# tl32rodan/DCVC

Hardware: AMD Instinct MI355X
Metric: encode+decode fps @1920x1080 per GPU; bpp bit-exact + PSNR Δ<1e-4 dB vs ref (higher is better)
Workload: dtype f32 (convs on split-fp16 f16x3 MFMA, fp32 accumulation); 1 GPU; C3 DCVC-DC RGB 1920x1080 (pad 1920x1088) IP=32 write mode; gop=32, precision=split, q_index=0, stream_part=8, parallelism=sequence-sharded x1, 3 GOP lane(s) per GPU, lanes=3, step=one frame on each of 3 lane(s)

## Files before the change

### dcvc_amd/csrc/hip/sdc.hip

```cpp
#include "common.h"
#include "launch.h"
#include "split.h"

namespace {

constexpr int kNW = 8, kNT = kNW * 64;
constexpr int TH = 8, TW = 16;
constexpr int HW_ = TW + 2, NPH = (TH + 2) * HW_;
constexpr int HR = 192;

struct DP {
  const float *x;
  int H, W, xcs, xco;
  float *y;
  int ycs, yco;
  const uint16_t *w;
  int wbytes;
  const float *b1, *wdw, *bdw, *b2, *ba;
  float slope;
  int tiles_x, ntiles;
  int *ovf;
};

template <int CIN, int COUT, bool ADAPT>
struct DG {
  static constexpr int KCI = (CIN + 31) / 32;
  static constexpr int NTI = (CIN + 15) / 16, NTO = (COUT + 15) / 16;
  static constexpr int CI16 = NTI * 16, CO16 = NTO * 16;
  static constexpr int W1 = KCI * CI16 * 32, W2 = KCI * CO16 * 32, WA = ADAPT ? KCI * CO16 * 32 : 0;
  static constexpr int NWH = 2 * (W1 + W2 + WA);
  static constexpr int XI = KCI * HR * 32;
  static constexpr int DI = KCI * TH * TW * 32;
  static constexpr size_t OX = 0, OD = OX + (size_t)2 * XI * 2, OW = OD + (size_t)2 * DI * 2;
  static constexpr size_t OC = OW + (size_t)NWH * 2;
  static constexpr int NC = CIN * 11 + 2 * COUT;
  static constexpr size_t LDS = OC + (size_t)NC * 4;
  static constexpr int QP = CIN / 8;
  static constexpr int PP = (NPH * QP + kNT - 1) / kNT;
};

__device__ __forceinline__ float lrelu(float v, float s) { return fmaxf(v, v * s); }

template <int CIN, int COUT, bool ADAPT>
__global__ void __launch_bounds__(kNT) sdc_kernel(DP p) {
  SplitRange rg(p.ovf);
  typedef DG<CIN, COUT, ADAPT> G_;
  constexpr int KCI = G_::KCI, NTI = G_::NTI, NTO = G_::NTO, CO16 = G_::CO16, CI16 = G_::CI16;
  constexpr int XI = G_::XI, DI = G_::DI, QP = G_::QP, PP = G_::PP;
  extern __shared__ __align__(16) unsigned char smem[];
  uint16_t *Xh = reinterpret_cast<uint16_t *>(smem + G_::OX), *Xl = Xh + XI;
  uint16_t *Dh = reinterpret_cast<uint16_t *>(smem + G_::OD), *Dl = Dh + DI;
  uint16_t *W1h = reinterpret_cast<uint16_t *>(smem + G_::OW), *W1l = W1h + G_::W1;
  uint16_t *W2h = W1l + G_::W1, *W2l = W2h + G_::W2;
  uint16_t *WAh = W2l + G_::W2, *WAl = WAh + G_::WA;
  float *Lb1 = reinterpret_cast<float *>(smem + G_::OC), *Lbdw = Lb1 + CIN, *Lwdw = Lbdw + CIN;
  float *Lb2 = Lwdw + 9 * CIN, *Lba = Lb2 + COUT;
  auto t1p = [&](int r, int c) -> float * {
    return reinterpret_cast<float *>((c & 16) ? Xl : Xh) + (((c >> 5) * HR + r) * 16 + (c & 15));
  };

  const int tid = threadIdx.x;
  const int wave = tid >> 6, lane = tid & 63;
  const int col = lane & 15, hi = lane >> 4;
  const int G = gridDim.x;
  int g = blockIdx.x;
  if ((G & 7) == 0) g = (g & 7) * (G >> 3) + (g >> 3);
  if (g >= p.ntiles) return;

  {
    const __amdgpu_buffer_rsrc_t wr =
        __builtin_amdgcn_make_buffer_rsrc(const_cast<uint16_t *>(p.w), (short)0, p.wbytes, 0x00020000);
    constexpr int ND = G_::NWH * 2 / 1024;
    for (int i = wave; i < ND; i += kNW)
      __builtin_amdgcn_raw_ptr_buffer_load_lds(wr, (__attribute__((address_space(3))) void *)(W1h + i * 512), 16,
                                               i * 1024 + lane * 16, 0, 0, 0);
    for (int i = tid; i < G_::NC; i += kNT) {
      float v;
      if (i < CIN) v = p.b1[i];
      else if (i < 2 * CIN) v = p.bdw[i - CIN];
      else if (i < 11 * CIN) v = p.wdw[i - 2 * CIN];
      else if (i < 11 * CIN + COUT) v = p.b2[i - 11 * CIN];
      else v = ADAPT ? p.ba[i - 11 * CIN - COUT] : 0.f;
      Lb1[i] = v;
    }
  }

  const __amdgpu_buffer_rsrc_t xr = __builtin_amdgcn_make_buffer_rsrc(
      const_cast<float *>(p.x), (short)0,
      (int)((int64_t)p.H * p.W * p.xcs * 4 < 0x7fff0000 ? (int64_t)p.H * p.W * p.xcs * 4 : 0x7fff0000), 0x00020000);
  int pyx[PP], prel[PP], pofs[PP];
#pragma unroll
  for (int u = 0; u < PP; ++u) {
    const int it = tid + u * kNT;
    pyx[u] = -1;
    prel[u] = 0;
    pofs[u] = 0;
    if (it < NPH * QP) {
      const int pix = it / QP, q = it - pix * QP;
      const int hy = pix / HW_, hx = pix - hy * HW_;
      pyx[u] = (hy << 8) | hx;
      prel[u] = ((hy - 1) * p.W + (hx - 1)) * p.xcs + p.xco + q * 8;
      pofs[u] = swz((q >> 2) * HR + pix, q & 3);
    }
  }
  float pf[PP][8];
  auto prefetch = [&](int t) {
    const int oy0 = (t / p.tiles_x) * TH, ox0 = (t % p.tiles_x) * TW;
    const int base = oy0 * p.W + ox0;
#pragma unroll
    for (int u = 0; u < PP; ++u) {
      const int gy = oy0 - 1 + (pyx[u] >> 8), gx = ox0 - 1 + (pyx[u] & 255);
      const bool in = pyx[u] >= 0 && (unsigned)gy < (unsigned)p.H && (unsigned)gx < (unsigned)p.W;
      const int o = in ? (base * p.xcs + prel[u]) * 4 : 0x7fffffe0;
      const f32x4 a = __builtin_bit_cast(f32x4, __builtin_amdgcn_raw_buffer_load_b128(xr, o, 0, 0));
      const f32x4 b = __builtin_bit_cast(f32x4, __builtin_amdgcn_raw_buffer_load_b128(xr, o + 16, 0, 0));
#pragma unroll
      for (int j = 0; j < 4; ++j) {
        pf[u][j] = a[j];
        pf[u][4 + j] = b[j];
      }
    }
  };
  prefetch(g);

  auto zero_pad = [&]() {
    if constexpr (CIN % 32 != 0) {
      constexpr int PADQ = KCI * 4 - QP;
      for (int it = tid; it < HR * PADQ; it += kNT) {
        const int row = it / PADQ, q = QP + it % PADQ;
        const int o = swz((q >> 2) * HR + row, q & 3);
        *reinterpret_cast<u32x4_t *>(Xh + o) = u32x4_t{0u, 0u, 0u, 0u};
        *reinterpret_cast<u32x4_t *>(Xl + o) = u32x4_t{0u, 0u, 0u, 0u};
      }
    }
  };

  wait_vm_lgkm();
  for (int t = g; t < p.ntiles; t += G) {
    const int oy0 = (t / p.tiles_x) * TH, ox0 = (t % p.tiles_x) * TW;
    raw_barrier();
#pragma unroll
    for (int u = 0; u < PP; ++u) {
      u32x4_t h, l;
      rg.add8(pf[u]);
      split8(pf[u], h, l);
      if (pyx[u] >= 0) {
        *reinterpret_cast<u32x4_t *>(Xh + pofs[u]) = h;
        *reinterpret_cast<u32x4_t *>(Xl + pofs[u]) = l;
      }
    }
    zero_pad();
    wait_lgkm();
    raw_barrier();
    if (t + G < p.ntiles) prefetch(t + G);

    f32x4 idn[NTO];
    if constexpr (ADAPT) {
      f32x4 am[NTO], ac[NTO];
#pragma unroll
      for (int j = 0; j < NTO; ++j) {
        am[j] = f32x4{0.f, 0.f, 0.f, 0.f};
        ac[j] = f32x4{0.f, 0.f, 0.f, 0.f};
      }
      const int hr = (wave + 1) * HW_ + 1 + col;
#pragma unroll
      for (int kc = 0; kc < KCI; ++kc) {
        const int ob = swz(kc * HR + hr, hi);
        const f16x8 bh = *reinterpret_cast<const f16x8 *>(Xh + ob), bl = *reinterpret_cast<const f16x8 *>(Xl + ob);
#pragma unroll
        for (int j = 0; j < NTO; ++j) {
          const int oa = swz(kc * CO16 + j * 16 + col, hi);
          const f16x8 ah = *reinterpret_cast<const f16x8 *>(WAh + oa), al = *reinterpret_cast<const f16x8 *>(WAl + oa);
          am[j] = __builtin_amdgcn_mfma_f32_16x16x32_f16(ah, bh, am[j], 0, 0, 0);
          ac[j] = __builtin_amdgcn_mfma_f32_16x16x32_f16(ah, bl, ac[j], 0, 0, 0);
          ac[j] = __builtin_amdgcn_mfma_f32_16x16x32_f16(al, bh, ac[j], 0, 0, 0);
        }
      }
#pragma unroll
      for (int j = 0; j < NTO; ++j) {
        const int n = j * 16 + hi * 4;
#pragma unroll
        for (int e = 0; e < 4; ++e) idn[j][e] = (am[j][e] + ac[j][e] * kLoInv) + Lba[n + e < COUT ? n + e : 0];
      }
      wait_lgkm();
      raw_barrier();
    }

    for (int ht = wave; ht < HR / 16; ht += kNW) {
      f32x4 tm[NTI], tc[NTI];
#pragma unroll
      for (int j = 0; j < NTI; ++j) {
        tm[j] = f32x4{0.f, 0.f, 0.f, 0.f};
        tc[j] = f32x4{0.f, 0.f, 0.f, 0.f};
      }
      const int r = ht * 16 + col;
#pragma unroll
      for (int kc = 0; kc < KCI; ++kc) {
        const int ob = swz(kc * HR + r, hi);
        const f16x8 bh = *reinterpret_cast<const f16x8 *>(Xh + ob), bl = *reinterpret_cast<const f16x8 *>(Xl + ob);
#pragma unroll
        for (int j = 0; j < NTI; ++j) {
          const int oa = swz(kc * CI16 + j * 16 + col, hi);
          const f16x8 ah = *reinterpret_cast<const f16x8 *>(W1h + oa), al = *reinterpret_cast<const f16x8 *>(W1l + oa);
          tm[j] = __builtin_amdgcn_mfma_f32_16x16x32_f16(ah, bh, tm[j], 0, 0, 0);
          tc[j] = __builtin_amdgcn_mfma_f32_16x16x32_f16(ah, bl, tc[j], 0, 0, 0);
          tc[j] = __builtin_amdgcn_mfma_f32_16x16x32_f16(al, bh, tc[j], 0, 0, 0);
        }
      }
      const int hy = r / HW_, hx = r - hy * HW_;
      const int gy = oy0 - 1 + hy, gx = ox0 - 1 + hx;
      const bool inside = r < NPH && (unsigned)gy < (unsigned)p.H && (unsigned)gx < (unsigned)p.W;
      wave_lds_sync();
#pragma unroll
      for (int j = 0; j < NTI; ++j) {
        const int n = j * 16 + hi * 4;
        if (n >= CIN) continue;
        f32x4 v;
#pragma unroll
        for (int e = 0; e < 4; ++e) v[e] = inside ? lrelu((tm[j][e] + tc[j][e] * kLoInv) + Lb1[n + e], p.slope) : 0.f;
        *reinterpret_cast<f32x4 *>(t1p(r, n)) = v;
      }
    }
    wait_lgkm();
    raw_barrier();

    {
      constexpr int CG = CIN / 4;
      constexpr int R = kNT / (CG * TW) >= 4 ? 4 : kNT / (CG * TW) >= 2 ? 2 : 1;
      constexpr int RR = TH / R;
      static_assert(CG * TW * R <= kNT && TH % R == 0, "P2 tasks");
      if (tid < CG * TW * R) {
        const int cg = tid % CG, rest = tid / CG;
        const int ix = rest % TW, y0 = (rest / TW) * RR;
        const int c = cg * 4;
        f32x4 wv[9];
#pragma unroll
        for (int k = 0; k < 9; ++k) wv[k] = *reinterpret_cast<const f32x4 *>(Lwdw + k * CIN + c);
        const float4 bd = *reinterpret_cast<const float4 *>(Lbdw + c);
        f32x4 win[3][3];
#pragma unroll
        for (int r = 0; r < 2; ++r)
#pragma unroll
          for (int dx = 0; dx < 3; ++dx)
            win[r][dx] = *reinterpret_cast<const f32x4 *>(t1p((y0 + r) * HW_ + ix + dx, c));
#pragma unroll
        for (int i = 0; i < RR; ++i) {
#pragma unroll
          for (int dx = 0; dx < 3; ++dx)
            win[(i + 2) % 3][dx] = *reinterpret_cast<const f32x4 *>(t1p((y0 + i + 2) * HW_ + ix + dx, c));
          f32x4 a = f32x4{0.f, 0.f, 0.f, 0.f};
#pragma unroll
          for (int dy = 0; dy < 3; ++dy)
#pragma unroll
            for (int dx = 0; dx < 3; ++dx)
#pragma unroll
              for (int e = 0; e < 4; ++e) a[e] = __builtin_fmaf(wv[dy * 3 + dx][e], win[(i + dy) % 3][dx][e], a[e]);
          float v[4];
          v[0] = a[0] + bd.x;
          v[1] = a[1] + bd.y;
          v[2] = a[2] + bd.z;
          v[3] = a[3] + bd.w;
          rg.add4(v);
          const auto h01 = __builtin_amdgcn_cvt_pkrtz(v[0], v[1]);
          const auto h23 = __builtin_amdgcn_cvt_pkrtz(v[2], v[3]);
          const uint32_t l01 = pk(split_lo(v[0], (float)h01[0]), split_lo(v[1], (float)h01[1]));
          const uint32_t l23 = pk(split_lo(v[2], (float)h23[0]), split_lo(v[3], (float)h23[1]));
          const int px = (y0 + i) * TW + ix;
          const int o = swz((c >> 5) * (TH * TW) + px, (c & 31) >> 3) + (c & 7);
          typedef unsigned int u32x2_t __attribute__((ext_vector_type(2)));
          *reinterpret_cast<u32x2_t *>(Dh + o) = u32x2_t{__builtin_bit_cast(uint32_t, h01), __builtin_bit_cast(uint32_t, h23)};
          *reinterpret_cast<u32x2_t *>(Dl + o) = u32x2_t{l01, l23};
        }
      }
      if constexpr (CIN % 32 != 0) {
        constexpr int PADQ = KCI * 4 - CIN / 8;
        for (int it = tid; it < TH * TW * PADQ; it += kNT) {
          const int px = it / PADQ, q = CIN / 8 + it % PADQ;
          const int o = swz((q >> 2) * (TH * TW) + px, q & 3);
          *reinterpret_cast<u32x4_t *>(Dh + o) = u32x4_t{0u, 0u, 0u, 0u};
          *reinterpret_cast<u32x4_t *>(Dl + o) = u32x4_t{0u, 0u, 0u, 0u};
        }
      }
    }
    wait_lgkm();
    raw_barrier();

    {
      f32x4 cm[NTO], cc[NTO];
#pragma unroll
      for (int j = 0; j < NTO; ++j) {
        cm[j] = f32x4{0.f, 0.f, 0.f, 0.f};
        cc[j] = f32x4{0.f, 0.f, 0.f, 0.f};
      }
#pragma unroll
      for (int kc = 0; kc < KCI; ++kc) {
        const int ob = swz(kc * (TH * TW) + wave * TW + col, hi);
        const f16x8 bh = *reinterpret_cast<const f16x8 *>(Dh + ob), bl = *reinterpret_cast<const f16x8 *>(Dl + ob);
#pragma unroll
        for (int j = 0; j < NTO; ++j) {
          const int oa = swz(kc * CO16 + j * 16 + col, hi);
          const f16x8 ah = *reinterpret_cast<const f16x8 *>(W2h + oa), al = *reinterpret_cast<const f16x8 *>(W2l + oa);
          cm[j] = __builtin_amdgcn_mfma_f32_16x16x32_f16(ah, bh, cm[j], 0, 0, 0);
          cc[j] = __builtin_amdgcn_mfma_f32_16x16x32_f16(ah, bl, cc[j], 0, 0, 0);
          cc[j] = __builtin_amdgcn_mfma_f32_16x16x32_f16(al, bh, cc[j], 0, 0, 0);
        }
      }
      const int gy = oy0 + wave, gx = ox0 + col;
      if (gy < p.H && gx < p.W) {
        const int64_t pix = (int64_t)gy * p.W + gx;
#pragma unroll
        for (int j = 0; j < NTO; ++j) {
          const int n = j * 16 + hi * 4;
          if (n >= COUT) continue;
          f32x4 id;
          if constexpr (ADAPT) id = idn[j];
          else id = *reinterpret_cast<const f32x4 *>(p.x + pix * p.xcs + p.xco + n);
          f32x4 v;
#pragma unroll
          for (int e = 0; e < 4; ++e) v[e] = ((cm[j][e] + cc[j][e] * kLoInv) + Lb2[n + e]) + id[e];
          *reinterpret_cast<f32x4 *>(p.y + pix * p.ycs + p.yco + n) = v;
        }
      }
    }
  }
  wait_vm_lgkm();
}

template <int CIN, int COUT, bool ADAPT>
int run(DP p, hipStream_t st) {
  typedef DG<CIN, COUT, ADAPT> G_;
  static_assert(G_::LDS <= 160 * 1024, "LDS");
  static_assert(G_::NWH * 2 % 1024 == 0, "weight images in whole 1-KiB pieces");
  p.tiles_x = (p.W + TW - 1) / TW;
  const int64_t nt = (int64_t)p.tiles_x * ((p.H + TH - 1) / TH);
  if (nt <= 0) return DCVC_HIP_OK;
  p.ntiles = (int)nt;
  const int cus = dcvc_cu_count();
  if (cus <= 0) return DCVC_HIP_ELAUNCH;
  int G = cus;
  if (G > p.ntiles) G = p.ntiles;
  auto kern = sdc_kernel<CIN, COUT, ADAPT>;
  dcvc_note_kernel("sdc_kernel<%d, %d, %s>@%lld", CIN, COUT, bname(ADAPT), (long long)G * kNT);
  dcvc_ensure_lds(reinterpret_cast<const void *>(kern), (int)G_::LDS);
  hipLaunchKernelGGL(kern, dim3((unsigned)G), dim3(kNT), G_::LDS, st, p);
  DCVC_LAUNCH_CHECK();
  return DCVC_HIP_OK;
}

bool supported(int cin, int cout, bool adapt) {
  return (cin == 64 && cout == 48 && adapt) || (cin == 48 && cout == 32 && adapt) ||
         (cin == 64 && cout == 64 && !adapt) || (cin == 32 && cout == 64 && adapt) ||
         (cin == 48 && cout == 48 && !adapt) || (cin == 32 && cout == 32 && !adapt);
}

}

extern "C" int64_t dcvc_dc_pack_weights(const float *w1, const float *w2, const float *wa, int cin, int cout,
                                        void *out) {
  if (!w1 || !w2 || cin <= 0 || cout <= 0) return DCVC_HIP_EINVAL;
  if (out && (!host_split_range_ok(w1, (int64_t)cin * cin) || !host_split_range_ok(w2, (int64_t)cout * cin) ||
              (wa && !host_split_range_ok(wa, (int64_t)cout * cin))))
    return DCVC_HIP_EINVAL;
  const int kci = (cin + 31) / 32, ci16 = (cin + 15) / 16 * 16, co16 = (cout + 15) / 16 * 16;
  const int64_t n1 = (int64_t)kci * ci16 * 32, n2 = (int64_t)kci * co16 * 32, na = wa ? n2 : 0;
  const int64_t total = 2 * (n1 + n2 + na);
  if (!out) return total;
  uint16_t *o = reinterpret_cast<uint16_t *>(out);
  auto at = [](int row, int k) {
    const int x = (0x1320 >> (((row >> 2) & 3) << 2)) & 3;
    return (int64_t)row * 32 + ((((k >> 3) ^ x) & 3) << 3) + (k & 7);
  };
  auto put = [&](uint16_t *img, int64_t n, const float *w, int rows, int rows16) {
    for (int kc = 0; kc < kci; ++kc)
      for (int r = 0; r < rows16; ++r)
        for (int k = 0; k < 32; ++k) {
          const int ch = kc * 32 + k;
          const float v = (r < rows && ch < cin) ? w[(int64_t)r * cin + ch] : 0.f;
          const int64_t q = at(kc * rows16 + r, k);
          host_split(v, img[q], img[n + q]);
        }
  };
  put(o, n1, w1, cin, ci16);
  put(o + 2 * n1, n2, w2, cout, co16);
  if (wa) put(o + 2 * n1 + 2 * n2, na, wa, cout, co16);
  return total;
}

extern "C" int dcvc_depth_conv_split(const dcvc_dc_args *a, void *stream) {
  if (!a || !a->x.ptr || !a->y.ptr || !a->w || !a->b1 || !a->wdw || !a->bdw || !a->b2) return DCVC_HIP_EINVAL;
  if (a->x.dtype != DCVC_F32 || a->y.dtype != DCVC_F32 || a->x.C != a->cin || a->y.C != a->cout ||
      a->x.H != a->y.H || a->x.W != a->y.W)
    return DCVC_HIP_EINVAL;
  const bool adapt = a->adaptor != 0;
  if (!supported(a->cin, a->cout, adapt) || (adapt && !a->ba)) return DCVC_HIP_EUNSUPPORTED;
  if (!(a->slope >= 0.f && a->slope <= 1.f)) return DCVC_HIP_EUNSUPPORTED;
  if (a->x.cstride % 4 || a->x.coff % 4 || a->y.cstride % 4 || a->y.coff % 4 || ((uintptr_t)a->x.ptr & 15) ||
      ((uintptr_t)a->y.ptr & 15))
    return DCVC_HIP_EUNSUPPORTED;
  if ((int64_t)a->x.H * a->x.W * a->x.cstride * 4 >= 0x7fff0000) return DCVC_HIP_EUNSUPPORTED;
  DP p{};
  p.ovf = dcvc_internal_split_flag();
  p.x = reinterpret_cast<const float *>(a->x.ptr);
  p.H = a->x.H;
  p.W = a->x.W;
  p.xcs = a->x.cstride;
  p.xco = a->x.coff;
  p.y = reinterpret_cast<float *>(a->y.ptr);
  p.ycs = a->y.cstride;
  p.yco = a->y.coff;
  p.w = reinterpret_cast<const uint16_t *>(a->w);
  p.wbytes = (int)(dcvc_dc_pack_weights(reinterpret_cast<const float *>(1), reinterpret_cast<const float *>(1),
                                        adapt ? reinterpret_cast<const float *>(1) : nullptr, a->cin, a->cout,
                                        nullptr) * 2);
  p.b1 = a->b1;
  p.wdw = a->wdw;
  p.bdw = a->bdw;
  p.b2 = a->b2;
  p.ba = a->ba;
  p.slope = a->slope;
  hipStream_t st = reinterpret_cast<hipStream_t>(stream);
  if (a->cin == 64 && a->cout == 48) return run<64, 48, true>(p, st);
  if (a->cin == 48 && a->cout == 32) return run<48, 32, true>(p, st);
  if (a->cin == 32 && a->cout == 64) return run<32, 64, true>(p, st);
  if (a->cin == 64 && a->cout == 64) return run<64, 64, false>(p, st);
  if (a->cin == 48 && a->cout == 48) return run<48, 48, false>(p, st);
  return run<32, 32, false>(p, st);
}
```

Before: 30.60 frames/s.

## Add software-pipelined depth-conv kernel overlapping conv1, depthwise and conv2 across channel groups

```diff
diff --git a/dcvc_amd/csrc/hip/sdc.h b/dcvc_amd/csrc/hip/sdc.h
--- /dev/null
+++ b/dcvc_amd/csrc/hip/sdc.h
@@ -0,0 +1,19 @@
+#pragma once
+#include <hip/hip_runtime.h>
+#include <stdint.h>
+
+struct SdcP {
+  const float *x;
+  int H, W, xcs, xco;
+  float *y;
+  int ycs, yco;
+  const uint16_t *w;
+  int wbytes;
+  const float *b1, *wdw, *bdw, *b2, *ba;
+  float slope;
+  int tiles_x, ntiles;
+  int *ovf;
+  int dbg;
+};
+
+int dcvc_internal_sdc_pipe(int cin, int cout, bool adapt, SdcP p, hipStream_t st);
diff --git a/dcvc_amd/csrc/hip/sdc.hip b/dcvc_amd/csrc/hip/sdc.hip
--- a/dcvc_amd/csrc/hip/sdc.hip
+++ b/dcvc_amd/csrc/hip/sdc.hip
@@ -1,5 +1,7 @@
 #include "common.h"
 #include "launch.h"
+#include "options.h"
+#include "sdc.h"
 #include "split.h"
 
 namespace {
@@ -9,18 +11,7 @@
 constexpr int HW_ = TW + 2, NPH = (TH + 2) * HW_;
 constexpr int HR = 192;
 
-struct DP {
-  const float *x;
-  int H, W, xcs, xco;
-  float *y;
-  int ycs, yco;
-  const uint16_t *w;
-  int wbytes;
-  const float *b1, *wdw, *bdw, *b2, *ba;
-  float slope;
-  int tiles_x, ntiles;
-  int *ovf;
-};
+typedef SdcP DP;
 
 template <int CIN, int COUT, bool ADAPT>
 struct DG {
@@ -44,6 +35,14 @@
 template <int CIN, int COUT, bool ADAPT>
 __global__ void __launch_bounds__(kNT) sdc_kernel(DP p) {
   SplitRange rg(p.ovf);
+#ifdef SDC_DBG
+  const int XD = p.dbg;
+#else
+  constexpr int XD = 0;
+#endif
+  auto barrier = [&]() __attribute__((always_inline)) {
+    if (!(XD & 128)) raw_barrier();
+  };
   typedef DG<CIN, COUT, ADAPT> G_;
   constexpr int KCI = G_::KCI, NTI = G_::NTI, NTO = G_::NTO, CO16 = G_::CO16, CI16 = G_::CI16;
   constexpr int XI = G_::XI, DI = G_::DI, QP = G_::QP, PP = G_::PP;
@@ -138,25 +137,26 @@
   wait_vm_lgkm();
   for (int t = g; t < p.ntiles; t += G) {
     const int oy0 = (t / p.tiles_x) * TH, ox0 = (t % p.tiles_x) * TW;
-    raw_barrier();
+    barrier();
 #pragma unroll
     for (int u = 0; u < PP; ++u) {
       u32x4_t h, l;
       rg.add8(pf[u]);
       split8(pf[u], h, l);
-      if (pyx[u] >= 0) {
+      if (pyx[u] >= 0 && !(XD & 1)) {
         *reinterpret_cast<u32x4_t *>(Xh + pofs[u]) = h;
         *reinterpret_cast<u32x4_t *>(Xl + pofs[u]) = l;
       }
     }
     zero_pad();
     wait_lgkm();
-    raw_barrier();
+    barrier();
     if (t + G < p.ntiles) prefetch(t + G);
 
     f32x4 idn[NTO];
     if constexpr (ADAPT) {
       f32x4 am[NTO], ac[NTO];
+      const int KA = (XD & 2) ? 0 : KCI;
 #pragma unroll
       for (int j = 0; j < NTO; ++j) {
         am[j] = f32x4{0.f, 0.f, 0.f, 0.f};
@@ -164,7 +164,7 @@
       }
       const int hr = (wave + 1) * HW_ + 1 + col;
 #pragma unroll
-      for (int kc = 0; kc < KCI; ++kc) {
+      for (int kc = 0; kc < KA; ++kc) {
         const int ob = swz(kc * HR + hr, hi);
         const f16x8 bh = *reinterpret_cast<const f16x8 *>(Xh + ob), bl = *reinterpret_cast<const f16x8 *>(Xl + ob);
 #pragma unroll
@@ -183,7 +183,7 @@
         for (int e = 0; e < 4; ++e) idn[j][e] = (am[j][e] + ac[j][e] * kLoInv) + Lba[n + e < COUT ? n + e : 0];
       }
       wait_lgkm();
-      raw_barrier();
+      barrier();
     }
 
     for (int ht = wave; ht < HR / 16; ht += kNW) {
@@ -194,8 +194,9 @@
         tc[j] = f32x4{0.f, 0.f, 0.f, 0.f};
       }
       const int r = ht * 16 + col;
-#pragma unroll
-      for (int kc = 0; kc < KCI; ++kc) {
+      const int K1 = (XD & 4) ? 0 : KCI;
+#pragma unroll
+      for (int kc = 0; kc < K1; ++kc) {
         const int ob = swz(kc * HR + r, hi);
         const f16x8 bh = *reinterpret_cast<const f16x8 *>(Xh + ob), bl = *reinterpret_cast<const f16x8 *>(Xl + ob);
 #pragma unroll
@@ -214,7 +215,7 @@
 #pragma unroll
       for (int j = 0; j < NTI; ++j) {
         const int n = j * 16 + hi * 4;
-        if (n >= CIN) continue;
+        if (n >= CIN || (XD & 8)) continue;
         f32x4 v;
 #pragma unroll
         for (int e = 0; e < 4; ++e) v[e] = inside ? lrelu((tm[j][e] + tc[j][e] * kLoInv) + Lb1[n + e], p.slope) : 0.f;
@@ -222,14 +223,14 @@
       }
     }
     wait_lgkm();
-    raw_barrier();
+    barrier();
 
     {
       constexpr int CG = CIN / 4;
       constexpr int R = kNT / (CG * TW) >= 4 ? 4 : kNT / (CG * TW) >= 2 ? 2 : 1;
       constexpr int RR = TH / R;
       static_assert(CG * TW * R <= kNT && TH % R == 0, "P2 tasks");
-      if (tid < CG * TW * R) {
+      if (tid < CG * TW * R && !(XD & 16)) {
         const int cg = tid % CG, rest = tid / CG;
         const int ix = rest % TW, y0 = (rest / TW) * RR;
         const int c = cg * 4;
@@ -283,7 +284,7 @@
       }
     }
     wait_lgkm();
-    raw_barrier();
+    barrier();
 
     {
       f32x4 cm[NTO], cc[NTO];
@@ -292,8 +293,9 @@
         cm[j] = f32x4{0.f, 0.f, 0.f, 0.f};
         cc[j] = f32x4{0.f, 0.f, 0.f, 0.f};
       }
-#pragma unroll
-      for (int kc = 0; kc < KCI; ++kc) {
+      const int K3 = (XD & 32) ? 0 : KCI;
+#pragma unroll
+      for (int kc = 0; kc < K3; ++kc) {
         const int ob = swz(kc * (TH * TW) + wave * TW + col, hi);
         const f16x8 bh = *reinterpret_cast<const f16x8 *>(Dh + ob), bl = *reinterpret_cast<const f16x8 *>(Dl + ob);
 #pragma unroll
@@ -306,7 +308,7 @@
         }
       }
       const int gy = oy0 + wave, gx = ox0 + col;
-      if (gy < p.H && gx < p.W) {
+      if (gy < p.H && gx < p.W && !(XD & 64)) {
         const int64_t pix = (int64_t)gy * p.W + gx;
 #pragma unroll
         for (int j = 0; j < NTO; ++j) {
@@ -346,6 +348,10 @@
   DCVC_LAUNCH_CHECK();
   return DCVC_HIP_OK;
 }
+
+#ifdef SDC_DBG
+DCVC_OPTION("sdc_dbg", g_dbg, 0);
+#endif
 
 bool supported(int cin, int cout, bool adapt) {
   return (cin == 64 && cout == 48 && adapt) || (cin == 48 && cout == 32 && adapt) ||
@@ -419,6 +425,12 @@
   p.ba = a->ba;
   p.slope = a->slope;
   hipStream_t st = reinterpret_cast<hipStream_t>(stream);
+#ifdef SDC_DBG
+  p.dbg = g_dbg;
+#else
+  const int rp = dcvc_internal_sdc_pipe(a->cin, a->cout, adapt, p, st);
+  if (rp != DCVC_HIP_EUNSUPPORTED) return rp;
+#endif
   if (a->cin == 64 && a->cout == 48) return run<64, 48, true>(p, st);
   if (a->cin == 48 && a->cout == 32) return run<48, 32, true>(p, st);
   if (a->cin == 32 && a->cout == 64) return run<32, 64, true>(p, st);
diff --git a/dcvc_amd/csrc/hip/sdcp.hip b/dcvc_amd/csrc/hip/sdcp.hip
--- /dev/null
+++ b/dcvc_amd/csrc/hip/sdcp.hip
@@ -0,0 +1,388 @@
+#include "common.h"
+#include "launch.h"
+#include "options.h"
+#include "sdc.h"
+#include "split.h"
+
+namespace {
+
+constexpr int kNW = 8, kNT = kNW * 64;
+constexpr int TH = 8, TW = 16;
+constexpr int HW_ = TW + 2, NPH = (TH + 2) * HW_;
+constexpr int HR = 192;
+constexpr int TP = TH * TW;
+constexpr int kOob = 0x7fffffe0;
+
+typedef uint32_t u32x2_t __attribute__((ext_vector_type(2)));
+
+template <int CIN, int COUT, bool ADAPT>
+struct PG {
+  static constexpr int KCI = (CIN + 31) / 32;
+  static constexpr int NTI = (CIN + 15) / 16, NTO = (COUT + 15) / 16;
+  static constexpr int CI16 = NTI * 16, CO16 = NTO * 16;
+  static constexpr int W1 = KCI * CI16 * 32, W2 = KCI * CO16 * 32, WA = ADAPT ? KCI * CO16 * 32 : 0;
+  static constexpr int XI = KCI * HR * 32;
+  static constexpr int DI = KCI * TP * 32;
+  static constexpr int TPI = 36;
+  static constexpr int TS = NPH * TPI;
+  static constexpr size_t OX = 0, OD = OX + (size_t)2 * XI * 2, OT = OD + (size_t)2 * DI * 2;
+  static constexpr size_t OW = OT + (size_t)2 * TS * 4;
+  static constexpr size_t OC = OW + (size_t)2 * W1 * 2;
+  static constexpr int NC = CIN * 11 + 2 * COUT;
+  static constexpr size_t LDS = OC + (size_t)NC * 4;
+  static constexpr int QP = CIN / 8;
+  static constexpr int PP = (NPH * QP + kNT - 1) / kNT;
+  static constexpr int NRB = NTO <= 2 ? 2 : 4;
+  static constexpr int NPB = TH / (kNW / NRB);
+  static_assert(COUT % 16 == 0 && CIN % 16 == 0 && NTO <= NRB, "whole channel tiles");
+  static_assert(LDS <= 160 * 1024, "LDS of a CU");
+  static_assert((2 * W1 * 2) % 1024 == 0, "conv1's images in whole 1-KiB pieces");
+};
+
+__device__ __forceinline__ float lrelu(float v, float s) { return fmaxf(v, v * s); }
+
+template <int CIN, int COUT, bool ADAPT>
+__global__ void __launch_bounds__(kNT) sdc_kernel_pipe(SdcP p) {
+  SplitRange rg(p.ovf);
+  typedef PG<CIN, COUT, ADAPT> G_;
+  constexpr int KCI = G_::KCI, NTI = G_::NTI, NTO = G_::NTO, CO16 = G_::CO16, CI16 = G_::CI16;
+  constexpr int XI = G_::XI, DI = G_::DI, QP = G_::QP, PP = G_::PP, NRB = G_::NRB, NPB = G_::NPB;
+  extern __shared__ __align__(16) unsigned char smem[];
+  uint16_t *Xh = reinterpret_cast<uint16_t *>(smem + G_::OX), *Xl = Xh + XI;
+  uint16_t *Dh = reinterpret_cast<uint16_t *>(smem + G_::OD), *Dl = Dh + DI;
+  float *Ts = reinterpret_cast<float *>(smem + G_::OT);
+  uint16_t *W1h = reinterpret_cast<uint16_t *>(smem + G_::OW), *W1l = W1h + G_::W1;
+  float *Lb1 = reinterpret_cast<float *>(smem + G_::OC), *Lbdw = Lb1 + CIN, *Lwdw = Lbdw + CIN;
+  float *Lb2 = Lwdw + 9 * CIN, *Lba = Lb2 + COUT;
+
+  const int tid = threadIdx.x, lane = tid & 63;
+  const int wave = __builtin_amdgcn_readfirstlane(tid >> 6);
+  const int col = lane & 15, hi = lane >> 4;
+  const int rb = wave % NRB, pb0 = (wave / NRB) * NPB;
+  const bool mm = rb < NTO;
+  const int n = rb * 16 + hi * 4;
+  const int G = gridDim.x;
+  int g = blockIdx.x;
+  if ((G & 7) == 0) g = (g & 7) * (G >> 3) + (g >> 3);
+  if (g >= p.ntiles) return;
+
+  const __amdgpu_buffer_rsrc_t wr =
+      __builtin_amdgcn_make_buffer_rsrc(const_cast<uint16_t *>(p.w), (short)0, p.wbytes, 0x00020000);
+  {
+    constexpr int ND = 2 * G_::W1 * 2 / 1024;
+    for (int i = wave; i < ND; i += kNW)
+      __builtin_amdgcn_raw_ptr_buffer_load_lds(wr, (__attribute__((address_space(3))) void *)(W1h + i * 512), 16,
+                                               i * 1024 + lane * 16, 0, 0, 0);
+    for (int i = tid; i < G_::NC; i += kNT) {
+      float v;
+      if (i < CIN) v = p.b1[i];
+      else if (i < 2 * CIN) v = p.bdw[i - CIN];
+      else if (i < 11 * CIN) v = p.wdw[i - 2 * CIN];
+      else if (i < 11 * CIN + COUT) v = p.b2[i - 11 * CIN];
+      else v = ADAPT ? p.ba[i - 11 * CIN - COUT] : 0.f;
+      Lb1[i] = v;
+    }
+    for (int i = tid; i < (2 * XI + 2 * DI) / 8; i += kNT)
+      reinterpret_cast<u32x4_t *>(Xh)[i] = u32x4_t{0u, 0u, 0u, 0u};
+  }
+  f16x8 w2h[KCI], w2l[KCI], wah[KCI], wal[KCI];
+#pragma unroll
+  for (int kc = 0; kc < KCI; ++kc) {
+    const int o = mm ? swz(kc * CO16 + rb * 16 + col, hi) * 2 : kOob;
+    const int o2 = mm ? o + 2 * G_::W1 * 2 : kOob;
+    w2h[kc] = __builtin_bit_cast(f16x8, __builtin_amdgcn_raw_buffer_load_b128(wr, o2, 0, 0));
+    w2l[kc] = __builtin_bit_cast(f16x8, __builtin_amdgcn_raw_buffer_load_b128(wr, mm ? o2 + G_::W2 * 2 : kOob, 0, 0));
+    if constexpr (ADAPT) {
+      const int oa = mm ? o + (2 * G_::W1 + 2 * G_::W2) * 2 : kOob;
+      wah[kc] = __builtin_bit_cast(f16x8, __builtin_amdgcn_raw_buffer_load_b128(wr, oa, 0, 0));
+      wal[kc] = __builtin_bit_cast(f16x8, __builtin_amdgcn_raw_buffer_load_b128(wr, mm ? oa + G_::WA * 2 : kOob, 0, 0));
+    } else {
+      wah[kc] = w2h[kc];
+      wal[kc] = w2l[kc];
+    }
+  }
+
+  const __amdgpu_buffer_rsrc_t xr = __builtin_amdgcn_make_buffer_rsrc(
+      const_cast<float *>(p.x), (short)0,
+      (int)((int64_t)p.H * p.W * p.xcs * 4 < 0x7fff0000 ? (int64_t)p.H * p.W * p.xcs * 4 : 0x7fff0000), 0x00020000);
+  int pyx[PP], prel[PP], pofs[PP];
+#pragma unroll
+  for (int u = 0; u < PP; ++u) {
+    const int it = tid + u * kNT;
+    pyx[u] = -1;
+    prel[u] = 0;
+    pofs[u] = 0;
+    if (it < NPH * QP) {
+      const int pix = it / QP, q = it - pix * QP;
+      const int hy = pix / HW_, hx = pix - hy * HW_;
+      pyx[u] = (hy << 8) | hx;
+      prel[u] = ((hy - 1) * p.W + (hx - 1)) * p.xcs + p.xco + q * 8;
+      pofs[u] = swz((q >> 2) * HR + pix, q & 3);
+    }
+  }
+  float pf[PP][8];
+  auto prefetch = [&](int t) __attribute__((always_inline)) {
+    const int oy0 = (t / p.tiles_x) * TH, ox0 = (t % p.tiles_x) * TW;
+    const int base = oy0 * p.W + ox0;
+#pragma unroll
+    for (int u = 0; u < PP; ++u) {
+      const int gy = oy0 - 1 + (pyx[u] >> 8), gx = ox0 - 1 + (pyx[u] & 255);
+      const bool in = pyx[u] >= 0 && (unsigned)gy < (unsigned)p.H && (unsigned)gx < (unsigned)p.W;
+      const int o = in ? (base * p.xcs + prel[u]) * 4 : kOob;
+      const f32x4 a = __builtin_bit_cast(f32x4, __builtin_amdgcn_raw_buffer_load_b128(xr, o, 0, 0));
+      const f32x4 b = __builtin_bit_cast(f32x4, __builtin_amdgcn_raw_buffer_load_b128(xr, o + 16, 0, 0));
+#pragma unroll
+      for (int j = 0; j < 4; ++j) {
+        pf[u][j] = a[j];
+        pf[u][4 + j] = b[j];
+      }
+    }
+  };
+  auto publish = [&]() __attribute__((always_inline)) {
+#pragma unroll
+    for (int u = 0; u < PP; ++u) {
+      u32x4_t h, l;
+      rg.add8(pf[u]);
+      split8(pf[u], h, l);
+      if (pyx[u] >= 0) {
+        *reinterpret_cast<u32x4_t *>(Xh + pofs[u]) = h;
+        *reinterpret_cast<u32x4_t *>(Xl + pofs[u]) = l;
+      }
+    }
+  };
+
+  int wq = wave;
+  const int lx = swz(col, hi);
+  const int tw = col * G_::TPI + hi * 4;
+  const int dq = tid & 7, dcx = (tid >> 3) & 15, drp = tid >> 7;
+  const int trd = (2 * drp * HW_ + dcx) * G_::TPI + dq * 4;
+  const int dwr = swz(2 * drp * TW + dcx, dq >> 1) + (dq & 1) * 4;
+  int ax[NPB];
+#pragma unroll
+  for (int i = 0; i < NPB; ++i) ax[i] = swz((pb0 + i + 1) * HW_ + 1 + col, hi);
+
+  auto conv1 = [&](int gr, int oy0, int ox0) __attribute__((always_inline)) {
+    const int ntg = NTI - 2 * gr >= 2 ? 2 : 1;
+    float *T = Ts + (gr & 1) * G_::TS;
+#pragma unroll
+    for (int i = 0; i < 3; ++i) {
+      const int task = wq + 8 * i;
+      if (task >= 12 * ntg) continue;
+      const int nt = task >= 12 ? 1 : 0, rt = task - 12 * nt;
+      const int j = 2 * gr + nt;
+      const int r = rt * 16 + col;
+      const int xb = lx + rt * 512, wb = lx + j * 512;
+      f32x4 tm = f32x4{0.f, 0.f, 0.f, 0.f}, tc = f32x4{0.f, 0.f, 0.f, 0.f};
+#pragma unroll
+      for (int kc = 0; kc < KCI; ++kc) {
+        const int ob = xb + kc * HR * 32;
+        const f16x8 bh = *reinterpret_cast<const f16x8 *>(Xh + ob), bl = *reinterpret_cast<const f16x8 *>(Xl + ob);
+        const int oa = wb + kc * CI16 * 32;
+        const f16x8 ah = *reinterpret_cast<const f16x8 *>(W1h + oa), al = *reinterpret_cast<const f16x8 *>(W1l + oa);
+        tm = __builtin_amdgcn_mfma_f32_16x16x32_f16(ah, bh, tm, 0, 0, 0);
+        tc = __builtin_amdgcn_mfma_f32_16x16x32_f16(ah, bl, tc, 0, 0, 0);
+        tc = __builtin_amdgcn_mfma_f32_16x16x32_f16(al, bh, tc, 0, 0, 0);
+      }
+      if (r < NPH) {
+        const int hy = r / HW_, hx = r - hy * HW_;
+        const int gy = oy0 - 1 + hy, gx = ox0 - 1 + hx;
+        const bool inside = (unsigned)gy < (unsigned)p.H && (unsigned)gx < (unsigned)p.W;
+        const f32x4 b = *reinterpret_cast<const f32x4 *>(Lb1 + j * 16 + hi * 4);
+        f32x4 v;
+#pragma unroll
+        for (int e = 0; e < 4; ++e) v[e] = inside ? lrelu((tm[e] + tc[e] * kLoInv) + b[e], p.slope) : 0.f;
+        *reinterpret_cast<f32x4 *>(T + tw + rt * 16 * G_::TPI + nt * 16) = v;
+      }
+    }
+  };
+
+  auto put4 = [&](int gr, int px, const float *v) __attribute__((always_inline)) {
+    rg.add4(v);
+    const auto h0 = __builtin_amdgcn_cvt_pkrtz(v[0], v[1]);
+    const auto h1 = __builtin_amdgcn_cvt_pkrtz(v[2], v[3]);
+    const uint32_t l0 = pk(split_lo(v[0], (float)h0[0]), split_lo(v[1], (float)h0[1]));
+    const uint32_t l1 = pk(split_lo(v[2], (float)h1[0]), split_lo(v[3], (float)h1[1]));
+    const int off = dwr + (gr * TP + px) * 32;
+    *reinterpret_cast<u32x2_t *>(Dh + off) = u32x2_t{__builtin_bit_cast(uint32_t, h0), __builtin_bit_cast(uint32_t, h1)};
+    *reinterpret_cast<u32x2_t *>(Dl + off) = u32x2_t{l0, l1};
+  };
+  auto depthwise = [&](int gr) __attribute__((always_inline)) {
+    const int c0 = gr * 32 + dq * 4;
+    if (c0 >= CIN) return;
+    const float *T = Ts + (gr & 1) * G_::TS + trd;
+    f32x4 wv[2][3];
+    float a0[4] = {0.f, 0.f, 0.f, 0.f}, a1[4] = {0.f, 0.f, 0.f, 0.f};
+#pragma unroll
+    for (int hr = 0; hr < 4; ++hr) {
+      if (hr < 3) {
+#pragma unroll
+        for (int dx = 0; dx < 3; ++dx)
+          wv[hr & 1][dx] = *reinterpret_cast<const f32x4 *>(Lwdw + (hr * 3 + dx) * CIN + c0);
+      }
+#pragma unroll
+      for (int dx = 0; dx < 3; ++dx) {
+        const f32x4 a = *reinterpret_cast<const f32x4 *>(T + (hr * HW_ + dx) * G_::TPI);
+        if (hr < 3) {
+#pragma unroll
+          for (int e = 0; e < 4; ++e) a0[e] = __builtin_fmaf(wv[hr & 1][dx][e], a[e], a0[e]);
+        }
+        if (hr > 0) {
+#pragma unroll
+          for (int e = 0; e < 4; ++e) a1[e] = __builtin_fmaf(wv[(hr - 1) & 1][dx][e], a[e], a1[e]);
+        }
+      }
+      sched_fence();
+    }
+    const f32x4 bd = *reinterpret_cast<const f32x4 *>(Lbdw + c0);
+    float v0[4], v1[4];
+#pragma unroll
+    for (int e = 0; e < 4; ++e) {
+      v0[e] = a0[e] + bd[e];
+      v1[e] = a1[e] + bd[e];
+    }
+    put4(gr, 0, v0);
+    put4(gr, TW, v1);
+  };
+
+  f32x4 cm[NPB], cc[NPB], idn[NPB];
+#pragma unroll
+  for (int i = 0; i < NPB; ++i) {
+    cm[i] = f32x4{0.f, 0.f, 0.f, 0.f};
+    cc[i] = f32x4{0.f, 0.f, 0.f, 0.f};
+    idn[i] = f32x4{0.f, 0.f, 0.f, 0.f};
+  }
+  auto conv2 = [&](int kc) __attribute__((always_inline)) {
+    if (!mm) return;
+#pragma unroll
+    for (int i = 0; i < NPB; ++i) {
+      const int o = lx + (kc * TP + (pb0 + i) * TW) * 32;
+      const f16x8 bh = *reinterpret_cast<const f16x8 *>(Dh + o), bl = *reinterpret_cast<const f16x8 *>(Dl + o);
+      cm[i] = __builtin_amdgcn_mfma_f32_16x16x32_f16(w2h[kc], bh, cm[i], 0, 0, 0);
+      cc[i] = __builtin_amdgcn_mfma_f32_16x16x32_f16(w2h[kc], bl, cc[i], 0, 0, 0);
+      cc[i] = __builtin_amdgcn_mfma_f32_16x16x32_f16(w2l[kc], bh, cc[i], 0, 0, 0);
+    }
+  };
+  auto adaptor = [&]() __attribute__((always_inline)) {
+    if (!mm) return;
+    const f32x4 bav = *reinterpret_cast<const f32x4 *>(Lba + n);
+#pragma unroll
+    for (int i = 0; i < NPB; ++i) {
+      f32x4 am = f32x4{0.f, 0.f, 0.f, 0.f}, ac = f32x4{0.f, 0.f, 0.f, 0.f};
+#pragma unroll
+      for (int kc = 0; kc < KCI; ++kc) {
+        const int ob = ax[i] + kc * HR * 32;
+        const f16x8 bh = *reinterpret_cast<const f16x8 *>(Xh + ob), bl = *reinterpret_cast<const f16x8 *>(Xl + ob);
+        am = __builtin_amdgcn_mfma_f32_16x16x32_f16(wah[kc], bh, am, 0, 0, 0);
+        ac = __builtin_amdgcn_mfma_f32_16x16x32_f16(wah[kc], bl, ac, 0, 0, 0);
+        ac = __builtin_amdgcn_mfma_f32_16x16x32_f16(wal[kc], bh, ac, 0, 0, 0);
+      }
+#pragma unroll
+      for (int e = 0; e < 4; ++e) idn[i][e] = (am[e] + ac[e] * kLoInv) + bav[e];
+    }
+  };
+  auto load_identity = [&](int oy0, int ox0) __attribute__((always_inline)) {
+    if (!mm) return;
+#pragma unroll
+    for (int i = 0; i < NPB; ++i) {
+      const int gy = oy0 + pb0 + i, gx = ox0 + col;
+      const bool ok = gy < p.H && gx < p.W;
+      idn[i] = __builtin_bit_cast(
+          f32x4, __builtin_amdgcn_raw_buffer_load_b128(xr, ok ? ((gy * p.W + gx) * p.xcs + p.xco + n) * 4 : kOob, 0, 0));
+    }
+  };
+  auto finish = [&](int oy0, int ox0) __attribute__((always_inline)) {
+    conv2(KCI - 1);
+    if (!mm) return;
+    const f32x4 b2v = *reinterpret_cast<const f32x4 *>(Lb2 + n);
+#pragma unroll
+    for (int i = 0; i < NPB; ++i) {
+      const int gy = oy0 + pb0 + i, gx = ox0 + col;
+      if (gy < p.H && gx < p.W) {
+        const int64_t pix = (int64_t)gy * p.W + gx;
+        f32x4 v;
+#pragma unroll
+        for (int e = 0; e < 4; ++e) v[e] = ((cm[i][e] + cc[i][e] * kLoInv) + b2v[e]) + idn[i][e];
+        *reinterpret_cast<f32x4 *>(p.y + pix * p.ycs + p.yco + n) = v;
+      }
+      cm[i] = f32x4{0.f, 0.f, 0.f, 0.f};
+      cc[i] = f32x4{0.f, 0.f, 0.f, 0.f};
+    }
+  };
+
+  prefetch(g);
+  wait_vm_lgkm();
+  raw_barrier();
+  publish();
+  if (g + G < p.ntiles) prefetch(g + G);
+  wait_lgkm();
+  raw_barrier();
+
+  int poy = 0, pox = 0;
+  for (int t = g; t < p.ntiles; t += G) {
+    const int oy0 = (t / p.tiles_x) * TH, ox0 = (t % p.tiles_x) * TW;
+    opaque_s(wq);
+#pragma unroll
+    for (int s = 0; s <= KCI; ++s) {
+      if (s == 0 && t != g) finish(poy, pox);
+      sched_fence();
+      if (s < KCI) conv1(s, oy0, ox0);
+      sched_fence();
+      if (ADAPT && s == KCI - 1) adaptor();
+      sched_fence();
+      if (s >= 2) conv2(s - 2);
+      sched_fence();
+      if (s >= 1) depthwise(s - 1);
+      sched_fence();
+      if (s == KCI) {
+        if (t + G < p.ntiles) {
+          publish();
+          if (t + 2 * G < p.ntiles) prefetch(t + 2 * G);
+        }
+        if (!ADAPT) load_identity(oy0, ox0);
+      }
+      wait_lgkm();
+      raw_barrier();
+    }
+    poy = oy0;
+    pox = ox0;
+  }
+  finish(poy, pox);
+}
+
+DCVC_OPTION("sdcpipe", g_pipe, 1);
+
+template <int CIN, int COUT, bool ADAPT>
+int run(SdcP p, hipStream_t st) {
+  typedef PG<CIN, COUT, ADAPT> G_;
+  p.tiles_x = (p.W + TW - 1) / TW;
+  const int64_t nt = (int64_t)p.tiles_x * ((p.H + TH - 1) / TH);
+  if (nt <= 0) return DCVC_HIP_OK;
+  p.ntiles = (int)nt;
+  const int cus = dcvc_cu_count();
+  if (cus <= 0) return DCVC_HIP_ELAUNCH;
+  int G = cus;
+  if (G > p.ntiles) G = p.ntiles;
+  auto kern = sdc_kernel_pipe<CIN, COUT, ADAPT>;
+  dcvc_note_kernel("sdc_kernel_pipe<%d, %d, %s>@%lld", CIN, COUT, bname(ADAPT), (long long)G * kNT);
+  dcvc_ensure_lds(reinterpret_cast<const void *>(kern), (int)G_::LDS);
+  hipLaunchKernelGGL(kern, dim3((unsigned)G), dim3(kNT), G_::LDS, st, p);
+  DCVC_LAUNCH_CHECK();
+  return DCVC_HIP_OK;
+}
+
+bool wins(int cin, int cout, bool adapt) {
+  return adapt && ((cin == 64 && cout == 48) || (cin == 48 && cout == 32) || (cin == 32 && cout == 64));
+}
+
+}
+
+int dcvc_internal_sdc_pipe(int cin, int cout, bool adapt, SdcP p, hipStream_t st) {
+  if (g_pipe <= 0 || (g_pipe == 1 && !wins(cin, cout, adapt))) return DCVC_HIP_EUNSUPPORTED;
+  if (cin == 64 && cout == 48 && adapt) return run<64, 48, true>(p, st);
+  if (cin == 48 && cout == 32 && adapt) return run<48, 32, true>(p, st);
+  if (cin == 32 && cout == 64 && adapt) return run<32, 64, true>(p, st);
+  if (cin == 64 && cout == 64 && !adapt) return run<64, 64, false>(p, st);
+  if (cin == 48 && cout == 48 && !adapt) return run<48, 48, false>(p, st);
+  if (cin == 32 && cout == 32 && !adapt) return run<32, 32, false>(p, st);
+  return DCVC_HIP_EUNSUPPORTED;
+}
```

New measurement: 30.83 frames/s, median of 4. About the same (+0.8%).
